# StevenWang30/R-PCC

Hardware: AMD Instinct MI355X
Metric: frames/s (64E, 64x2048 range img), projection->segmentation->model->quantise (higher is better)
Workload: dtype f32

## Files before the change

r-pcc_amd/csrc/rpcc_hip.hip:

```cpp
#include <hip/hip_runtime.h>
#include <limits.h>
#include <math.h>
#include <stdint.h>
#include <stdio.h>
#include <string.h>

#include <algorithm>
#include <mutex>
#include <new>
#include <type_traits>
#include <utility>
#include <vector>
#include "../../include/rpcc_hip.h"
#include "rpcc_device.h"
#include "ref_rules.h"

using namespace rpcc;

static thread_local char g_err[512] = "";
static int set_err(int code, const char *fmt, const char *a = "", const char *b = "") {
    snprintf(g_err, sizeof(g_err), fmt, a, b);
    return code;
}
#define HIP_TRY(expr)                                                                      \
// ... 2281 lines not shown
#pragma unroll
        for (int e = 0; e < ASSIGN_PX; e++) unknown |= live[e] && !(tp[e] >= 0.0f);
        if (__ballot(unknown) == 0ull) {
#pragma unroll
            for (int e = 0; e < ASSIGN_PX; e++) reach = fmaxf(reach, live[e] ? (tp[e] < 1e10f ? tp[e] : inf) : 0.0f);
        } else {
#pragma unroll
            for (int e = 0; e < ASSIGN_PX; e++) reach = fmaxf(reach, live[e] ? assign_reach(r[e], tx[e], ty[e], tz[e], tp[e] < 1e10f ? tp[e] : -1.0f, G) : 0.0f);
        }
        reach = dpp_max_f32_native(reach);
        const bool bounded = reach < inf;
        float my_dmin[NR], upper = inf;
#pragma unroll
        for (int rd = 0; rd < NR; rd++) {
            const int k = rd * 64 + lane;
            my_dmin[rd] = inf;
            if (rd * 64 < M && k < M) {
                const float4 cc = cen4[k];
                const float a0 = lo0 - cc.x, b0 = cc.x - hi0, a1 = lo1 - cc.y, b1 = cc.y - hi1, a2 = lo2 - cc.z, b2 = cc.z - hi2;
                const float g0 = fmaxf(fmaxf(a0, b0), 0.0f), g1 = fmaxf(fmaxf(a1, b1), 0.0f), g2 = fmaxf(fmaxf(a2, b2), 0.0f);
                my_dmin[rd] = (g0 * g0 + g1 * g1) + g2 * g2;
                if (!bounded) {
                    const float f0 = fmaxf(fabsf(a0), fabsf(b0)), f1 = fmaxf(fabsf(a1), fabsf(b1)), f2 = fmaxf(fabsf(a2), fabsf(b2));
                    upper = fminf(upper, (f0 * f0 + f1 * f1) + f2 * f2);
                }
            }
        }
        if (!bounded) upper = dpp_min_f32_native(upper);
        const float cut = (bounded ? reach : upper) * 1.000002f;
        unsigned long long surv_m[NR], surv_any = 0ull;
#pragma unroll
        for (int rd = 0; rd < NR; rd++) { surv_m[rd] = rd * 64 < M ? __ballot(my_dmin[rd] <= cut) : 0ull; surv_any |= surv_m[rd]; }
        if (surv_any == 0ull) {
#pragma unroll
            for (int e = 0; e < ASSIGN_PX; e++)
                if (valid[e]) st_at(seg_b, (uint32_t)p[e] * (uint32_t)sizeof(L), (L)(r[e] == 0.0f ? 1 : 0));
            continue;
        }
        float m1[ASSIGN_PX], m2[ASSIGN_PX];
        int k1[ASSIGN_PX];
        rs_v2f xv[ASSIGN_PX / 2], yv[ASSIGN_PX / 2], zv[ASSIGN_PX / 2];
#pragma unroll
        for (int e = 0; e < ASSIGN_PX; e++) { m1[e] = inf; m2[e] = inf; k1[e] = -1; }
#pragma unroll
        for (int e2 = 0; e2 < ASSIGN_PX / 2; e2++) {
            xv[e2] = rs_v2f{x[2 * e2], x[2 * e2 + 1]}; yv[e2] = rs_v2f{y[2 * e2], y[2 * e2 + 1]}; zv[e2] = rs_v2f{z[2 * e2], z[2 * e2 + 1]};
        }
#pragma unroll
        for (int rd = 0; rd < NR; rd++) {
            if (rd * 64 >= M) break;
            unsigned long long surv = surv_m[rd];
            while (surv) {
                const int k = rd * 64 + (int)__ffsll((long long)surv) - 1;
                surv &= surv - 1ull;
                const float4 cc = cen4[k];
#pragma unroll
                for (int e2 = 0; e2 < ASSIGN_PX / 2; e2++) {
                    const rs_v2f dx = xv[e2] - rs_v2f{cc.x, cc.x}, dy = yv[e2] - rs_v2f{cc.y, cc.y}, dz = zv[e2] - rs_v2f{cc.z, cc.z};
                    const rs_v2f dd = (dx * dx + dy * dy) + dz * dz;
#pragma unroll
                    for (int e1 = 0; e1 < 2; e1++) {
                        const int e = 2 * e2 + e1;
                        const float d2 = e1 ? dd.y : dd.x;
                        const bool lt = d2 < m1[e];
                        m2[e] = __builtin_amdgcn_fmed3f(m1[e], m2[e], d2);
                        k1[e] = lt ? k : k1[e];
                        m1[e] = lt ? d2 : m1[e];
                    }
                }
            }
        }
        int lab[ASSIGN_PX];
#pragma unroll
        for (int e = 0; e < ASSIGN_PX; e++) {
            lab[e] = assign_label(r[e], tx[e], ty[e], tz[e], x[e], y[e], z[e], m1[e], m2[e], k1[e], cen4, G);
            if (r[e] == 0.0f) lab[e] = 1;
            if (valid[e]) st_at(seg_b, (uint32_t)p[e] * (uint32_t)sizeof(L), (L)lab[e]);
        }
        if constexpr (SUMS) {
            int todo[ASSIGN_PX];
#pragma unroll
            for (int e = 0; e < ASSIGN_PX; e++) todo[e] = lab[e] >= 2 ? lab[e] : -1;
            static_assert(ASSIGN_PX == 4, "four pixel slots: round_label");
            uint32_t lo[ASSIGN_PX], hi[ASSIGN_PX];
            bool inexact = false;
            unsigned long long pend[ASSIGN_PX];
#pragma unroll
            for (int e = 0; e < ASSIGN_PX; e++) {
                lo[e] = hi[e] = 0u;
                if (todo[e] >= 2) inexact |= !range_fixed(f2u(r[e]), lo[e], hi[e]);
                pend[e] = __ballot(todo[e] >= 2);
            }
#pragma unroll 1
            while ((pend[0] | pend[1] | pend[2] | pend[3]) != 0ull) {
                const int cur = round_label(todo, pend);
                uint32_t slo = 0u, shi = 0u;
#pragma unroll
                for (int e = 0; e < ASSIGN_PX; e++) {
                    const bool mine = todo[e] == cur;
                    pend[e] &= ~__ballot(mine);
                    slo += mine ? lo[e] : 0u;
                    shi += mine ? hi[e] : 0u;
                }
                slo = dpp_sum_u32(slo); shi = dpp_sum_u32(shi);
                if (lane == 0)
                    atomicAdd(reinterpret_cast<unsigned long long *>(&acc.sums[(int64_t)b * acc.KP + cur]), (unsigned long long)slo + ((unsigned long long)shi << 18));
            }
            if (__any(inexact) && lane == 0) acc.flags[4 * b] = 1;
        }
    }
}

static inline int kpad(int M);
template <class L, class S>
static void launch_assign_form(const float *ri, const float *tm, const double *ground, const float *centers, int B, int H, int W, int M, L *seg,
                               hipStream_t st, const float *temp, const S acc) {
    const int ntile = ((H + ASSIGN_ROWS - 1) / ASSIGN_ROWS) * ((W + 31) / 32);
    const dim3 grid((ntile + ASSIGN_WAVES * ASSIGN_TILES_PER_WAVE - 1) / (ASSIGN_WAVES * ASSIGN_TILES_PER_WAVE), B);
    const size_t sh = (size_t)M * sizeof(float4);
    if constexpr (sizeof(L) == 1) assign_kernel<L, 4><<<grid, 64 * ASSIGN_WAVES, sh, st>>>(ri, tm, ground, centers, H, W, M, seg, temp, acc);
    else if (M <= 510)            assign_kernel<L, 8><<<grid, 64 * ASSIGN_WAVES, sh, st>>>(ri, tm, ground, centers, H, W, M, seg, temp, acc);
    else                          assign_kernel<L, 16><<<grid, 64 * ASSIGN_WAVES, sh, st>>>(ri, tm, ground, centers, H, W, M, seg, temp, acc);
}
template <class L>
static int launch_assign(const float *ri, const float *tm, const double *ground, const float *centers, int B, int H,
                         int W, int M, L *seg, hipStream_t st, const float *temp = nullptr, int64_t *sums = nullptr, int32_t *flags = nullptr) {
    ARG_TRY((sums == nullptr) == (flags == nullptr));
    if (sums != nullptr) launch_assign_form(ri, tm, ground, centers, B, H, W, M, seg, st, temp, LabelSums{sums, flags, kpad(M)});
    else                 launch_assign_form(ri, tm, ground, centers, B, H, W, M, seg, st, temp, NoSums{});
    LAUNCH_CHECK();
    return RPCC_OK;
}

template <class L>
static int assign_entry(const float *ri, const float *tm, const double *ground, const float *centers, int B, int H, int W, int M, L *seg,
                        void *stream) {
    ARG_TRY(B > 0 && B <= RPCC_MAX_BATCH && H > 0 && W > 0 && M > 0 && M <= LabelTraits<L>::max_clusters && ri && tm && ground && centers && seg);
    return launch_assign(ri, tm, ground, centers, B, H, W, M, seg, (hipStream_t)stream);
}
extern "C" int rpcc_assign(const float *ri, const float *tm, const double *ground, const float *centers, int B, int H, int W, int M, uint8_t *seg,
                           void *stream) {
    return assign_entry(ri, tm, ground, centers, B, H, W, M, seg, stream);
}
extern "C" int rpcc_assign_wide(const float *ri, const float *tm, const double *ground, const float *centers, int B, int H, int W, int M, uint16_t *seg,
                                void *stream) {
    return assign_entry(ri, tm, ground, centers, B, H, W, M, seg, stream);
}

#define TILE 1024
#define FX_UNIT_LOG2 28

static inline int kpad(int M) { return ((M + 2) + 63) & ~63; }
static inline int ntiles(int P) { return (P + TILE - 1) / TILE; }
struct WsLayout {
    int64_t *sums;
    int32_t *flags;
    uint32_t *hist;
    size_t bytes;
};
static WsLayout ws_layout(void *ws, int B, int P, int M) {
    const size_t KP = (size_t)kpad(M), T = (size_t)ntiles(P);
    Carve c(ws);
    WsLayout L;
    L.sums = c.take<int64_t>((size_t)B * KP * 8); L.flags = c.take<int32_t>((size_t)B * 4 * 4); L.hist = c.take<uint32_t>((size_t)B * T * KP * 4);
    L.bytes = c.bytes();
    return L;
}
struct PlaneLayout { uint32_t *order; float4 *pts4; size_t bytes; };
static PlaneLayout plane_layout(void *extra, int B, int P) {
    Carve c(extra);
    uint32_t *order = c.take<uint32_t>((size_t)B * P * 4);
    float4 *pts4 = c.take<float4>((size_t)B * P * 16);
    return {order, pts4, c.bytes()};
}
struct BatchLayout {
    WsLayout L;
    int32_t *epoch, *kpn = nullptr; char *proj_scratch, *extra = nullptr; float *temp, *rays_soa, *tiletab, *label_acc = nullptr;
    size_t proj_bytes, bytes;
};
static BatchLayout batch_layout(void *ws, int B, int P, int M, int64_t total_points, bool general) {
    Carve c(ws);
    BatchLayout l;
    l.L = ws_layout(ws, B, P, M); c.take(l.L.bytes); l.epoch = c.take<int32_t>(256);
    l.proj_bytes = round_up(project_layout(nullptr, total_points, B, P).bytes, 256); l.proj_scratch = c.take(l.proj_bytes);
    l.temp = c.take<float>((size_t)B * P * 4);
    l.rays_soa = c.take<float>((size_t)3 * P * 4 + 256, 4);
    l.tiletab = c.take<float>(0, 4);
    const size_t tab_bytes = fps_tab_bound_bytes(B, P), ksz = round_up((size_t)B * (M + 2) * 4, 256);
    Carve t(l.tiletab);
    t.take(tab_bytes + 256);
    if (general) {
        l.extra = t.take(plane_layout(nullptr, B, P).bytes);
        l.kpn = t.take<int32_t>(ksz, 4); l.label_acc = t.take<float>(ksz, 4); t.take(256, 1);
    }
    char *handoff_end = reinterpret_cast<char *>(wc_slot_of(rs_wc_of(reinterpret_cast<int32_t *>(l.tiletab), B, P), B, B).cnt);
    l.bytes = handoff_end <= reinterpret_cast<char *>(l.tiletab) + tab_bytes ? c.bytes() + t.bytes() : 0;
    return l;
}
static size_t batch_ws_bytes(int B, int P, int M, int64_t total_points, bool general) {
    const size_t n = B > 0 && P > 0 && M > 0 ? batch_layout(nullptr, B, P, M, total_points, general).bytes : 0;
    return n ? n + 4096 : 0;
}
extern "C" size_t rpcc_workspace_bytes(int B, int P, int M, int64_t total_points) { return batch_ws_bytes(B, P, M, total_points, false); }
extern "C" size_t rpcc_workspace_bytes_general(int B, int P, int M, int64_t total_points) { return batch_ws_bytes(B, P, M, total_points, true); }

#define SCAN_U 16
#define SCAN_THREADS 256
struct ScanArgs {
    const float *ri;
    const uint8_t *seg;
    const double *ground;
    int P, M, KP, T, KP2;
    const int64_t *sums;
    const int32_t *flags;
    uint32_t *hist;
    float *model;
    int32_t *counts, *nnz;
};
__device__ __forceinline__ void model_scan_body(const ScanArgs &A, const int b) {
    const float *__restrict__ ri = A.ri;
    const uint8_t *__restrict__ seg = A.seg;
    const double *__restrict__ ground = A.ground;
    const int P = A.P, M = A.M, KP = A.KP, T = A.T, KP2 = A.KP2;
    const int64_t *__restrict__ sums = A.sums;
    const int32_t *__restrict__ flags = A.flags;
    uint32_t *__restrict__ hist = A.hist;
    float *__restrict__ model = A.model;
    int32_t *__restrict__ counts = A.counts, *__restrict__ nnz = A.nnz;
    __shared__ uint32_t gtot[SCAN_THREADS];
    __shared__ uint32_t base[256];
    __shared__ uint32_t wsum[4];
    const int K = M + 2;
    const int NG = SCAN_THREADS / KP2, k = threadIdx.x & (KP2 - 1), grp = threadIdx.x / KP2;
    const int TG = (T + NG - 1) / NG, tbeg = grp * TG, tend = min(T, tbeg + TG);
    uint32_t *gh = hist + (int64_t)b * T * KP;
    const uint32_t kp4 = (uint32_t)KP * 4u, k4 = (uint32_t)k * 4u;
    const bool held = TG <= SCAN_U;
    uint32_t c[SCAN_U];
    uint32_t part = 0;
    if (k < K) {
        if (held) {
#pragma unroll
            for (int j = 0; j < SCAN_U; j++) c[j] = ld_at(gh, (uint32_t)min(tbeg + j, T - 1) * kp4 + k4);
#pragma unroll
            for (int j = 0; j < SCAN_U; j++) { if (tbeg + j >= tend) c[j] = 0u; part += c[j]; }
        } else {
            for (int t0 = tbeg; t0 < tend; t0 += SCAN_U) {
                uint32_t d[SCAN_U];
#pragma unroll
                for (int j = 0; j < SCAN_U; j++) d[j] = ld_at(gh, (uint32_t)min(t0 + j, T - 1) * kp4 + k4);
#pragma unroll
                for (int j = 0; j < SCAN_U; j++) part += t0 + j < tend ? d[j] : 0u;
            }
        }
    }
    gtot[grp * KP2 + k] = k < K ? part : 0u;
    __syncthreads();
    uint32_t total = 0;
    for (int g2 = 0; g2 < NG; g2++) total += gtot[g2 * KP2 + k];
    {
        const int kk = threadIdx.x;
        uint32_t v = 0u;
        if (kk < 256 && kk < K && kk != 1) { for (int g2 = 0; g2 < NG; g2++) v += gtot[g2 * KP2 + kk]; }
        const uint32_t incl = dpp_scan_incl_u32(v);
        if (kk < 256 && (kk & 63) == 63) wsum[kk >> 6] = incl;
        __syncthreads();
        if (kk < 256) {
            uint32_t off = 0u;
            for (int w = 0; w < (kk >> 6); w++) off += wsum[w];
            base[kk] = off + incl - v;
            if (kk == 255 && nnz) nnz[b] = (int32_t)(off + incl);
        }
    }
    __syncthreads();
    if (k < K) {
        uint32_t run = base[k];
        for (int g2 = 0; g2 < grp; g2++) run += gtot[g2 * KP2 + k];
        if (held) {
#pragma unroll
            for (int j = 0; j < SCAN_U; j++) {
                if (tbeg + j < tend) { st_at(gh, (uint32_t)(tbeg + j) * kp4 + k4, run); run += c[j]; }
            }
        } else {
            for (int t0 = tbeg; t0 < tend; t0 += SCAN_U) {
                uint32_t d[SCAN_U];
#pragma unroll
                for (int j = 0; j < SCAN_U; j++) d[j] = ld_at(gh, (uint32_t)min(t0 + j, T - 1) * kp4 + k4);
#pragma unroll
                for (int j = 0; j < SCAN_U; j++) {
                    if (t0 + j < tend) { st_at(gh, (uint32_t)(t0 + j) * kp4 + k4, run); run += d[j]; }
                }
            }
        }
        if (counts && grp == 0) counts[(int64_t)b * K + k] = (int32_t)total;
    }
    if (k < K && grp == 0 && model != nullptr)
        point_model_row(model, ground, flags, seg, ri, P, K, b, k, (long long)sums[(int64_t)b * KP + k], total);
}
__global__ __launch_bounds__(SCAN_THREADS) void model_scan_kernel(const ScanArgs A) { model_scan_body(A, blockIdx.x); }
__global__ __launch_bounds__(SCAN_THREADS) void model_scan_multi_kernel(const MultiArgs<ScanArgs> m) {
    int b, t;
    const ScanArgs &A = multi_locate(m, b, t);
    model_scan_body(A, b);
}
#define SCANW_THREADS 1024
template <class L>
__global__ __launch_bounds__(SCANW_THREADS) void model_scan_wide_kernel(const float *__restrict__ ri, const L *__restrict__ seg, const double *__restrict__ ground,
                                                                        int P, int M, int KP, int T, const int64_t *__restrict__ sums,
                                                                        const int32_t *__restrict__ flags, uint32_t *__restrict__ hist,
                                                                        float *__restrict__ model, int32_t *__restrict__ counts, int32_t *__restrict__ nnz) {
    __shared__ uint32_t wsum[SCANW_THREADS / 64];
    const int b = blockIdx.x, k = threadIdx.x, K = M + 2, lane = k & 63, wave = k >> 6;
    uint32_t *gh = hist + (int64_t)b * T * KP;
    const uint32_t kp4 = (uint32_t)KP * 4u, k4 = (uint32_t)min(k, KP - 1) * 4u;
    uint32_t total = 0u;
    for (int t0 = 0; t0 < T; t0 += SCAN_U) {
        uint32_t d[SCAN_U];
#pragma unroll
        for (int j = 0; j < SCAN_U; j++) d[j] = ld_at(gh, (uint32_t)min(t0 + j, T - 1) * kp4 + k4);
#pragma unroll
        for (int j = 0; j < SCAN_U; j++) total += (t0 + j < T && k < K) ? d[j] : 0u;
    }
    const uint32_t v = (k < K && k != 1) ? total : 0u;
    const uint32_t incl = dpp_scan_incl_u32(v);
    if (lane == 63) wsum[wave] = incl;
    __syncthreads();
    uint32_t off = 0u;
    for (int w = 0; w < wave; w++) off += wsum[w];
    if (k == SCANW_THREADS - 1 && nnz) nnz[b] = (int32_t)(off + incl);
    if (k >= K) return;
    uint32_t run = off + incl - v;
    for (int t0 = 0; t0 < T; t0 += SCAN_U) {
        uint32_t d[SCAN_U];
#pragma unroll
        for (int j = 0; j < SCAN_U; j++) d[j] = ld_at(gh, (uint32_t)min(t0 + j, T - 1) * kp4 + k4);
#pragma unroll
        for (int j = 0; j < SCAN_U; j++)
            if (t0 + j < T) { st_at(gh, (uint32_t)(t0 + j) * kp4 + k4, run); run += d[j]; }
    }
    if (counts) counts[(int64_t)b * K + k] = (int32_t)total;
    if (model != nullptr)
        point_model_row(model, ground, flags, seg, ri, P, K, b, k, (long long)sums[(int64_t)b * KP + k], total);
}
template <bool SUMS>
__device__ __forceinline__ void hist_aggregate(const int (&lab)[4], const uint32_t (&rb)[4], const int nval, int KP, int T, int64_t *__restrict__ sums,
                                               int32_t *__restrict__ flags, uint32_t *__restrict__ hist, const int b, const int t);
template <bool VEC, class L = uint8_t, bool SUMS = true>
__device__ __forceinline__ void model_hist_body(const float *__restrict__ ri, const L *__restrict__ seg,
                                                int P, int KP, int T, int64_t *__restrict__ sums,
                                                int32_t *__restrict__ flags, uint32_t *__restrict__ hist, const int b, const int t) {
    const L *seg_b = seg + (int64_t)b * P;
    const float *ri_b = SUMS ? ri + (int64_t)b * P : nullptr;
    const int p0 = t * TILE + 4 * (int)threadIdx.x;
    const int nval = min(max(P - p0, 0), 4);
    int lab[4];
    uint32_t rb[4];
    if (VEC) {
        const uint32_t q = (uint32_t)(nval > 0 ? p0 : 0);
        load_labels4(seg_b, q, lab);
        if constexpr (SUMS) {
            const uint4 r4 = ld_at(reinterpret_cast<const uint4 *>(ri_b), q * 4u);
            rb[0] = r4.x; rb[1] = r4.y; rb[2] = r4.z; rb[3] = r4.w;
        }
    } else {
#pragma unroll
        for (int e = 0; e < 4; e++) {
            const uint32_t gp = (uint32_t)min(p0 + e, P - 1);
            lab[e] = ld_at(seg_b, gp * (uint32_t)sizeof(L));
            if constexpr (SUMS) rb[e] = f2u(ld_at(ri_b, gp * 4u));
        }
    }
    hist_aggregate<SUMS>(lab, rb, nval, KP, T, sums, flags, hist, b, t);
}
template <bool SUMS>
__device__ __forceinline__ void hist_aggregate(const int (&lab)[4], const uint32_t (&rb)[4], const int nval, int KP, int T, int64_t *__restrict__ sums,
                                               int32_t *__restrict__ flags, uint32_t *__restrict__ hist, const int b, const int t) {
    extern __shared__ __attribute__((aligned(16))) unsigned char smem_raw[];
    unsigned long long *ssum = reinterpret_cast<unsigned long long *>(smem_raw);
    uint32_t *scnt = reinterpret_cast<uint32_t *>(SUMS ? smem_raw + (size_t)KP * 8 : smem_raw);
    const int lane = threadIdx.x & 63;
    for (int k = threadIdx.x; k < KP; k += blockDim.x) {
        if constexpr (SUMS) ssum[k] = 0ull;
        scnt[k] = 0u;
    }
    __syncthreads();
    bool inexact = false;
    int todo[4];
    uint32_t lo[4], hi[4];
#pragma unroll
    for (int e = 0; e < 4; e++) {
        todo[e] = e < nval ? lab[e] : -1;
        lo[e] = hi[e] = 0u;
        if constexpr (SUMS) {
            if (todo[e] >= 2) inexact |= !range_fixed(rb[e], lo[e], hi[e]);
        }
    }
#define HIST_ROUNDS 3
    unsigned long long pend[4];
#pragma unroll
    for (int e = 0; e < 4; e++) pend[e] = __ballot(todo[e] >= 0);
#pragma unroll 1
    for (int round = 0; round < HIST_ROUNDS && (pend[0] | pend[1] | pend[2] | pend[3]) != 0ull; round++) {
        const int cur = round_label(todo, pend);
        int ctot = 0;
        uint32_t slo = 0u, shi = 0u;
#pragma unroll
        for (int e = 0; e < 4; e++) {
            const bool mine = todo[e] == cur;
            const unsigned long long m = __ballot(mine);
            ctot += (int)__popcll(m);
            pend[e] &= ~m;
            if constexpr (SUMS) { slo += mine ? lo[e] : 0u; shi += mine ? hi[e] : 0u; }
        }
        const bool sum = SUMS && cur >= 2;
        if (sum) { slo = dpp_sum_u32(slo); shi = dpp_sum_u32(shi); }
        if (lane == 0) {
            atomicAdd(&scnt[cur], (uint32_t)ctot);
            if (sum) atomicAdd(&ssum[cur], (unsigned long long)slo + ((unsigned long long)shi << 18));
        }
    }
#pragma unroll
    for (int e = 0; e < 4; e++) {
        if (pend[e] != 0ull && ((pend[e] >> lane) & 1ull)) {
            atomicAdd(&scnt[todo[e]], 1u);
            if constexpr (SUMS) {
                if (todo[e] >= 2) atomicAdd(&ssum[todo[e]], (unsigned long long)lo[e] + ((unsigned long long)hi[e] << 18));
            }
        }
    }
    if constexpr (SUMS) {
        if (__any(inexact) && lane == 0) flags[4 * b] = 1;
    }
    __syncthreads();
    for (int k = threadIdx.x; k < KP; k += blockDim.x) {
        hist[((int64_t)b * T + t) * KP + k] = scnt[k];
        if constexpr (SUMS) {
            if (ssum[k]) atomicAdd(reinterpret_cast<unsigned long long *>(&sums[(int64_t)b * KP + k]), ssum[k]);
        }
    }
}
template <bool VEC, class L = uint8_t, bool SUMS = true>
__global__ __launch_bounds__(256) void model_hist_kernel(const float *__restrict__ ri, const L *__restrict__ seg,
                                                         int P, int KP, int T, int64_t *__restrict__ sums,
                                                         int32_t *__restrict__ flags, uint32_t *__restrict__ hist) {
    model_hist_body<VEC, L, SUMS>(ri, seg, P, KP, T, sums, flags, hist, blockIdx.y, blockIdx.x);
}
struct HistGroup {
    const uint8_t *seg;
    int P, T, vec;
    uint32_t *hist;
};
__global__ __launch_bounds__(256) void model_hist_multi_kernel(const MultiArgs<HistGroup> m, int KP) {
    int b, t;
    const HistGroup &a = multi_locate(m, b, t);
    if (a.vec) model_hist_body<true, uint8_t, false>(nullptr, a.seg, a.P, KP, a.T, nullptr, nullptr, a.hist, b, t);
    else       model_hist_body<false, uint8_t, false>(nullptr, a.seg, a.P, KP, a.T, nullptr, nullptr, a.hist, b, t);
}
static inline size_t hist_lds_bytes(int KP, bool sums) { return (sums ? (size_t)KP * 8 : 0) + (size_t)KP * 4; }
template <class L>
static inline bool hist_vec(int P, const L *seg, const float *ri) { return (P & 3) == 0 && seg4_aligned(seg) && (ri == nullptr || aligned16(ri)); }
static inline int scan_kp2(int M) { int v = 1; while (v < M + 2) v <<= 1; return v; }
template <class L>
static int launch_hist_scan(const float *ri, const L *seg, const double *ground, int B, int P, int M, const WsLayout &lay, float *model,
                            int32_t *counts, int32_t *nnz, hipStream_t st, bool summed = false, bool counted = false) {
    const int KP = kpad(M), T = ntiles(P);
    const bool hist_sums = ri != nullptr && !summed;
    const size_t sh = hist_lds_bytes(KP, hist_sums);
    const bool vec = hist_vec(P, seg, hist_sums ? ri : nullptr);
    if (counted) {
    } else if (hist_sums) {
        if (vec) model_hist_kernel<true, L, true><<<dim3(T, B), 256, sh, st>>>(ri, seg, P, KP, T, lay.sums, lay.flags, lay.hist);
        else     model_hist_kernel<false, L, true><<<dim3(T, B), 256, sh, st>>>(ri, seg, P, KP, T, lay.sums, lay.flags, lay.hist);
    } else {
        if (vec) model_hist_kernel<true, L, false><<<dim3(T, B), 256, sh, st>>>(nullptr, seg, P, KP, T, nullptr, nullptr, lay.hist);
        else     model_hist_kernel<false, L, false><<<dim3(T, B), 256, sh, st>>>(nullptr, seg, P, KP, T, nullptr, nullptr, lay.hist);
    }
    LAUNCH_CHECK();
    if constexpr (sizeof(L) == 1) {
        const ScanArgs sa = {ri, seg, ground, P, M, KP, T, scan_kp2(M), lay.sums, lay.flags, lay.hist, model, counts, nnz};
        model_scan_kernel<<<B, SCAN_THREADS, 0, st>>>(sa);
    } else {
        model_scan_wide_kernel<L><<<B, SCANW_THREADS, 0, st>>>(ri, seg, ground, P, M, KP, T, lay.sums, lay.flags, lay.hist, model, counts, nnz);
    }
    LAUNCH_CHECK();
    return RPCC_OK;
}

template <class L>
static int launch_point_model(const float *ri, const L *seg, const double *ground, int B, int P, int M,
                              float *model, int32_t *counts, int32_t *nnz, void *ws, hipStream_t st, bool cleared = false, bool summed = false,
                              bool counted = false) {
    const WsLayout lay = ws_layout(ws, B, P, M);
    if (!cleared) HIP_TRY(hipMemsetAsync(lay.sums, 0, (size_t)((char *)lay.hist - (char *)lay.sums), st));
    return launch_hist_scan(ri, seg, ground, B, P, M, lay, model, counts, nnz, st, summed, counted);
}

template <class L>
static int point_model_entry(const float *ri, const L *seg, const double *ground, int B, int P, int M, float *model, int32_t *counts,
                             void *ws, void *stream) {
    ARG_TRY(B > 0 && B <= RPCC_MAX_BATCH && P > 0 && M > 0 && M <= LabelTraits<L>::max_clusters && ri && seg && ground && model && ws);
    return launch_point_model(ri, seg, ground, B, P, M, model, counts, nullptr, ws, (hipStream_t)stream);
}
extern "C" int rpcc_point_model(const float *ri, const uint8_t *seg, const double *ground, int B, int P, int M, float *model, int32_t *counts, void *ws,
                                void *stream) {
    return point_model_entry(ri, seg, ground, B, P, M, model, counts, ws, stream);
}
extern "C" int rpcc_point_model_wide(const float *ri, const uint16_t *seg, const double *ground, int B, int P, int M, float *model, int32_t *counts, void *ws,
                                     void *stream) {
    return point_model_entry(ri, seg, ground, B, P, M, model, counts, ws, stream);
}

__device__ __forceinline__ void segment_prefix(uint32_t *segcnt, int SEGP, const uint32_t *tile_off, int K) {
    const int row = threadIdx.x >> 4, sgi = threadIdx.x & 15;
    for (int k0 = 0; k0 < K; k0 += 16) {
        const int k = k0 + row;
        const bool ok = k < K;
        const uint32_t c = ok ? segcnt[sgi * SEGP + k] : 0u;
        uint32_t v = c;
        v += (uint32_t)__builtin_amdgcn_update_dpp(0, (int)v, 0x111, 0xf, 0xf, false);
        v += (uint32_t)__builtin_amdgcn_update_dpp(0, (int)v, 0x112, 0xf, 0xf, false);
        v += (uint32_t)__builtin_amdgcn_update_dpp(0, (int)v, 0x114, 0xf, 0xf, false);
        v += (uint32_t)__builtin_amdgcn_update_dpp(0, (int)v, 0x118, 0xf, 0xf, false);
        if (ok) segcnt[sgi * SEGP + k] = tile_off[k] + v - c;
    }
}
__device__ __forceinline__ int segment_rank(int j, int lab, uint32_t *segcnt, int SEGP) {
    const int lane = threadIdx.x & 63, wave = threadIdx.x >> 6;
    int rank = 0, todo = lab;
    while (true) {
        const unsigned long long pending = __ballot(todo >= 0);
        if (!pending) break;
        const int leader = (int)__ffsll((long long)pending) - 1;
        const int cur = __builtin_amdgcn_readlane(todo, leader);
        const unsigned long long same = __ballot(todo == cur);
        if (todo == cur) {
            rank = __popcll(same & ((1ull << lane) - 1ull));
            if (lane == leader) segcnt[(j * 4 + wave) * SEGP + cur] = (uint32_t)__popcll(same);
            todo = -1;
        }
    }
    return rank;
}
__device__ __forceinline__ void segment_offsets(uint32_t *segcnt, int SEGP, const uint32_t *tile_off, int K) {
    __syncthreads();
    segment_prefix(segcnt, SEGP, tile_off, K);
    __syncthreads();
}
__device__ __forceinline__ uint32_t segment_slot(int j, int lab, int rank, const uint32_t *segcnt, int SEGP) {
    return segcnt[(j * 4 + (int)(threadIdx.x >> 6)) * SEGP + lab] + (uint32_t)rank;
}
static inline size_t segment_lds_bytes(int KP) { return (size_t)16 * (KP + 1) * 4 + (size_t)KP * 4; }

template <bool RESIDUAL_ONLY, bool VEC, class L = uint8_t>
__device__ __forceinline__ void predict_quantize_body(const float *__restrict__ ri, const float *__restrict__ tm,
                                                      const L *__restrict__ seg,
                                                      const float *__restrict__ model,
                                                      const uint32_t *__restrict__ hist, float acc,
                                                      const float *__restrict__ label_acc,
                                                      const float *__restrict__ residual_in, int P, int M,
                                                      int KP, int T, int16_t *__restrict__ q16,
                                                      int32_t *__restrict__ q32, float *__restrict__ pred_out,
                                                      int32_t *__restrict__ epoch_inc, const int b, const int t) {
    extern __shared__ __attribute__((aligned(16))) unsigned char smem_raw[];
    if (epoch_inc && b == 0 && t == 0 && threadIdx.x == 0) *epoch_inc += 1;
    float4 *smodel = reinterpret_cast<float4 *>(smem_raw);
    uint32_t *wcnt = reinterpret_cast<uint32_t *>(smodel + KP);
    uint32_t *soff = wcnt + 4 * KP;
    float *sacc = reinterpret_cast<float *>(soff + KP);
    const int K = M + 2;
    const int lane = threadIdx.x & 63, wave = threadIdx.x >> 6;
    seg += (int64_t)b * P;
    if (!RESIDUAL_ONLY) ri += (int64_t)b * P;
    if (residual_in) residual_in += (int64_t)b * P;
    if (pred_out) pred_out += (int64_t)b * P;
    if (q16) q16 += (int64_t)b * P;
    if (q32) q32 += (int64_t)b * P;
    if (label_acc) label_acc += (int64_t)b * K;
    if (!RESIDUAL_ONLY) model += (int64_t)b * K * 4;
    hist += ((int64_t)b * T + t) * KP;
    const int p0 = t * TILE + 4 * (int)threadIdx.x;
    const int nval = min(max(P - p0, 0), 4);
    int lab[4];
    float rv[4], ray[12], rin[4];
    if (VEC) {
        const uint32_t q = (uint32_t)(nval > 0 ? p0 : 0);
        load_labels4(seg, q, lab);
        if (RESIDUAL_ONLY) {
#pragma unroll
            for (int e = 0; e < 4; e++) rv[e] = 0.0f;
#pragma unroll
            for (int i = 0; i < 12; i++) ray[i] = 0.0f;
        } else {
            const float4 r4 = ld_at(reinterpret_cast<const float4 *>(ri), q * 4u);
            rv[0] = r4.x; rv[1] = r4.y; rv[2] = r4.z; rv[3] = r4.w;
            const float4 a = ld_at(reinterpret_cast<const float4 *>(tm), q * 12u), bq = ld_at(reinterpret_cast<const float4 *>(tm), q * 12u + 16u),
                         c = ld_at(reinterpret_cast<const float4 *>(tm), q * 12u + 32u);
            ray[0] = a.x; ray[1] = a.y; ray[2] = a.z; ray[3] = a.w; ray[4] = bq.x; ray[5] = bq.y; ray[6] = bq.z; ray[7] = bq.w;
            ray[8] = c.x; ray[9] = c.y; ray[10] = c.z; ray[11] = c.w;
        }
        if (residual_in) {
            const float4 x4 = ld_at(reinterpret_cast<const float4 *>(residual_in), q * 4u);
            rin[0] = x4.x; rin[1] = x4.y; rin[2] = x4.z; rin[3] = x4.w;
        } else {
            rin[0] = rin[1] = rin[2] = rin[3] = 0.0f;
        }
    } else {
#pragma unroll
        for (int e = 0; e < 4; e++) {
            const uint32_t up = (uint32_t)min(p0 + e, P - 1);
            lab[e] = ld_at(seg, up * (uint32_t)sizeof(L));
            rv[e] = RESIDUAL_ONLY ? 0.0f : ld_at(ri, up * 4u);
            if (RESIDUAL_ONLY) { ray[3 * e] = ray[3 * e + 1] = ray[3 * e + 2] = 0.0f; }
            else { ray[3 * e] = ld_f32(tm, up * 12u); ray[3 * e + 1] = ld_f32(tm, up * 12u + 4u); ray[3 * e + 2] = ld_f32(tm, up * 12u + 8u); }
            rin[e] = residual_in ? ld_at(residual_in, up * 4u) : 0.0f;
        }
    }
    for (uint32_t i = threadIdx.x; i < (uint32_t)K; i += 256u) {
        smodel[i] = RESIDUAL_ONLY ? make_float4(0.f, 0.f, 0.f, 0.f) : make_float4(model[4 * i], model[4 * i + 1], model[4 * i + 2], model[4 * i + 3]);
        soff[i] = hist[i];
        if (label_acc) sacc[i] = label_acc[i];
        wcnt[i] = 0u; wcnt[KP + i] = 0u; wcnt[2 * KP + i] = 0u; wcnt[3 * KP + i] = 0u;
// ... 426 lines not shown
                                 io->counts, p.ws, p.extra, st);
    case ST_QUANTISE:
        if (io->nonuniform) {
            const rpcc_nonuniform_cfg *nu = io->nonuniform;
            if ((rc = launch_features(io->ri, seg, Bs, p.g.H, p.g.W, nu->feature_region, nu->segments, nu->sharp_num, nu->less_sharp_num,
                                      nu->flat_num, nullptr, io->key_point_map, st, p.kpn, M + 2)))
                return rc;
            if ((rc = launch_salience_levels<L>(io->counts, p.kpn, Bs, M, salience_params(nu->levels, nu->level_kp_num, nu->level_acc, nu->ground_level),
                                                io->salience, p.label_acc, st)))
                return rc;
        }
        return launch_predict_quantize(io->ri, io->tm, seg, io->model, p.acc, p.label_acc, nullptr, Bs, P, M, io->q16,
                                       nullptr, nullptr, p.ws, st, p.epoch);
    }
    return RPCC_ERR_ARG;
}

static int check_batch_io(const rpcc_batch_io *io, int B, rpcc_geom g, int M, const void *ws, bool wide = false) {
    ARG_TRY(io != nullptr && ws != nullptr && B > 0 && B <= RPCC_MAX_BATCH && M > 0 && M <= (wide ? RPCC_MAX_CLUSTERS_WIDE : RPCC_MAX_CLUSTERS) &&
            g.H > 1 && g.W > 0);
    ARG_TRY(io->offsets && io->tm && io->ground && io->ri && io->seg && io->cen_pix && io->centers && io->model &&
            io->counts && io->q16 && io->nnz && io->info);
    ARG_TRY((io->flags & ~(RPCC_FPS_BRUTEFORCE | RPCC_FPS_MODE_BITS)) == 0);
    const int P = g.H * g.W;
    if (wide)
        ARG_TRY(!(io->flags & RPCC_FPS_MODE_BITS));
    else
        ARG_TRY(P % 4 == 0 || fps_pick_range(g.H, g.W, B, io->flags, true, true).family != FPS_ONE_PASS);
    ARG_TRY(io->model_method == 0 || io->model_method == 1);
    ARG_TRY(point_floats(io->point_stride_bytes) > 0 && (io->point_stride_bytes != 16 || (reinterpret_cast<uintptr_t>(io->xyz) & 15u) == 0));
    if (io->nonuniform) {
        const rpcc_nonuniform_cfg *nu = io->nonuniform;
        ARG_TRY(io->salience && io->key_point_map && nu->levels >= 1 && nu->levels <= 8 && nu->ground_level >= 0 && nu->ground_level < nu->levels);
    }
    return RPCC_OK;
}

template <class L>
static int run_batch(const rpcc_batch_io *io, int B, rpcc_geom g, int M, double ground_threshold, float acc, void *ws, int stage_mask, hipStream_t st,
                     const void *beams = nullptr) {
    BatchPlan p;
    int rc;
    if ((rc = plan_batch(p, io, B, io->total, g, M, ground_threshold, acc, reinterpret_cast<char *>(ws)))) return rc;
    p.beams = beams;
    for (int stage = 0; stage < ST_COUNT; stage++)
        if (((stage_mask >> stage) & 1) && (rc = run_stage<L>(p, stage, st))) return rc;
    return RPCC_OK;
}

extern "C" int rpcc_compress_batch(const rpcc_batch_io *io, int B, rpcc_geom g, int M, double ground_threshold,
                                   float acc, void *ws, void *stream) {
    int rc;
    if ((rc = check_batch_io(io, B, g, M, ws))) return rc;
    return run_batch<uint8_t>(io, B, g, M, ground_threshold, acc, ws, (1 << ST_COUNT) - 1, (hipStream_t)stream);
}

extern "C" int rpcc_compress_batch_stages(const rpcc_batch_io *io, int B, rpcc_geom g, int M, double ground_threshold, float acc, void *ws,
                                          int stage_mask, void *stream) {
    int rc;
    if ((rc = check_batch_io(io, B, g, M, ws))) return rc;
    return run_batch<uint8_t>(io, B, g, M, ground_threshold, acc, ws, stage_mask, (hipStream_t)stream);
}

static int mixed_ground(const BatchPlan *pl, int G, hipStream_t st) {
    RansacMulti m;
    m.n = 0; m.first[0] = 0;
    for (int i = 0; i < G; i++) {
        if (!pl[i].fit_ground) continue;
        const rpcc_batch_io *io = pl[i].io;
        m.a[m.n] = {io->ri, io->tm, pl[i].P, (uint32_t)io->ground_seed, io->ground, pl[i].zcnt, io->frame_ids,
                    pl[i].zcnt ? rs_wc_of(pl[i].zcnt, pl[i].Bs, pl[i].P) : nullptr, 100};
        m.first[m.n + 1] = m.first[m.n] + pl[i].Bs;
        m.n++;
    }
    if (m.n == 0) return RPCC_OK;
    return launch_ground_ransac_multi(m, st);
}
static int mixed_fps(const BatchPlan *pl, int G, hipStream_t st) {
    int rc, total = 0, tt = FPS_TT_SMALL;
    for (int i = 0; i < G; i++)
        if (pl[i].tiled && pl[i].io->timer == nullptr) total += pl[i].Bs;
    bool common[RPCC_MAX_GROUPS];
    FpsMulti m;
    m.n = 0; m.first[0] = 0;
    for (int i = 0; i < G; i++) {
        const BatchPlan &p = pl[i];
        const FpsPick k = fps_pick_range(p.g.H, p.g.W, total, p.io->flags, range_quads16(p.g.W, p.io->ri, p.temp, p.io->tm), true);
        common[i] = k.family == FPS_PLANAR && p.io->timer == nullptr;
        if (!common[i]) continue;
        tt = k.threads;
        m.a[m.n] = {p.io->ri, p.io->tm, p.temp, p.io->info, fps_tiling_range(p.g.H, p.g.W), p.io->cen_pix, p.io->centers, p.tiletab, p.rays_soa};
        m.edge[m.n] = k.unaligned ? 1 : 0;
        m.first[m.n + 1] = m.first[m.n] + p.Bs;
        m.n++;
    }
    if (m.n > 0) {
        if (tt == FPS_TT_SMALL) fps_regtab_planar_multi_kernel<FPS_TT_SMALL><<<m.first[m.n], FPS_TT_SMALL, 0, st>>>(m, pl[0].M, 0);
        else                    fps_regtab_planar_multi_kernel<FPS_TT_BATCH><<<m.first[m.n], FPS_TT_BATCH, 0, st>>>(m, pl[0].M, 0);
        LAUNCH_CHECK();
    }
    for (int i = 0; i < G; i++)
        if (!common[i] && (rc = run_stage<uint8_t>(pl[i], ST_FPS, st))) return rc;
    return RPCC_OK;
}
static int mixed_planes(const BatchPlan *pl, int G, hipStream_t st) {
    PlaneMulti m;
    m.n = 0; m.first[0] = 0;
    const int M = pl[0].M, K = M + 2, wpg = PL_THREADS / 64, groups = (K + wpg - 1) / wpg;
    for (int i = 0; i < G; i++) {
        const BatchPlan &p = pl[i];
        if (p.io->model_method == 0) continue;
        m.a[m.n] = plane_group_args(p.io->tm, p.io->ground, p.Bs, p.P, M, p.io->plane_cos_cut, (uint32_t)p.io->plane_seed, p.io->frame_ids,
                                    p.io->model, p.io->counts, p.ws, p.extra, nullptr);
        m.first[m.n + 1] = m.first[m.n] + p.Bs * (K - 2) + p.Bs * groups;
        m.n++;
    }
    if (m.n == 0) return RPCC_OK;
    plane_model_multi_kernel<10><<<m.first[m.n], PL_THREADS, 0, st>>>(m, M, kpad(M), PL_BIG);
    LAUNCH_CHECK();
    return RPCC_OK;
}

template <class A>
static void multi_add(MultiArgs<A> &m, const A &a, int frames, int per_frame) {
    m.a[m.n] = a; m.per[m.n] = per_frame; m.first[m.n + 1] = m.first[m.n] + frames * per_frame; m.n++;
}
static int mixed_assign(const BatchPlan *pl, int G, hipStream_t st) {
    int rc;
    for (int i = 0; i < G; i++) {
        const rpcc_batch_io *io = pl[i].io;
        const bool point = io->model_method == 0;
        if ((rc = launch_assign(io->ri, io->tm, io->ground, io->centers, pl[i].Bs, pl[i].g.H, pl[i].g.W, pl[i].M, io->seg, st,
                                (io->flags & RPCC_FPS_MODE_BITS) ? nullptr : pl[i].temp, point ? pl[i].L.sums : nullptr,
                                point ? pl[i].L.flags : nullptr))) return rc;
    }
    return RPCC_OK;
}
static int mixed_labels(const BatchPlan *pl, int G, hipStream_t st) {
    const int M = pl[0].M, KP = kpad(M);
    MultiArgs<HistGroup> mh; MultiArgs<ScanArgs> ms; MultiArgs<OrderGroup> mo;
    mh.n = ms.n = mo.n = 0; mh.first[0] = ms.first[0] = mo.first[0] = 0;
    for (int i = 0; i < G; i++) {
        const BatchPlan &p = pl[i];
        const rpcc_batch_io *io = p.io;
        const int T = ntiles(p.P);
        const bool point = io->model_method == 0;
        const float *ri = point ? io->ri : nullptr;
        multi_add(mh, HistGroup{io->seg, p.P, T, hist_vec(p.P, io->seg, (const float *)nullptr) ? 1 : 0, p.L.hist}, p.Bs, T);
        multi_add(ms, ScanArgs{ri, io->seg, point ? io->ground : nullptr, p.P, M, KP, T, scan_kp2(M), p.L.sums, p.L.flags, p.L.hist,
                               point ? io->model : nullptr, io->counts, io->nnz}, p.Bs, 1);
        const PlaneLayout pa = plane_layout(p.extra, p.Bs, p.P);
        if (!point) multi_add(mo, OrderGroup{io->seg, p.L.hist, p.P, T, pa.order, io->ri, io->tm, pa.pts4}, p.Bs, T);
    }
    model_hist_multi_kernel<<<mh.first[mh.n], 256, hist_lds_bytes(KP, false), st>>>(mh, KP);
    LAUNCH_CHECK();
    model_scan_multi_kernel<<<ms.first[ms.n], SCAN_THREADS, 0, st>>>(ms);
    LAUNCH_CHECK();
    if (mo.n > 0) {
        label_order_multi_kernel<<<mo.first[mo.n], 256, label_order_lds_bytes(KP), st>>>(mo, M, KP);
        LAUNCH_CHECK();
    }
    return RPCC_OK;
}
static int mixed_quantise(const BatchPlan *pl, int G, hipStream_t st) {
    int rc;
    const int M = pl[0].M, KP = kpad(M);
    MultiArgs<SalienceGroup> msal; MultiArgs<QuantGroup> mq;
    msal.n = mq.n = 0; msal.first[0] = mq.first[0] = 0;
    for (int i = 0; i < G; i++) {
        const BatchPlan &p = pl[i];
        const rpcc_batch_io *io = p.io;
        if (io->nonuniform) {
            const rpcc_nonuniform_cfg *nu = io->nonuniform;
            if ((rc = launch_features(io->ri, io->seg, p.Bs, p.g.H, p.g.W, nu->feature_region, nu->segments, nu->sharp_num, nu->less_sharp_num,
                                      nu->flat_num, nullptr, io->key_point_map, st, p.kpn, M + 2)))
                return rc;
            multi_add(msal, SalienceGroup{io->counts, p.kpn, salience_params(nu->levels, nu->level_kp_num, nu->level_acc, nu->ground_level), io->salience,
                                          p.label_acc}, p.Bs, 1);
        }
        const int T = ntiles(p.P);
        const bool vec = quantise_vec(p.P, io->seg, io->ri, io->tm, nullptr, false);
        multi_add(mq, QuantGroup{io->ri, io->tm, io->model, p.label_acc, io->seg, p.L.hist, p.P, T, vec ? 1 : 0, io->q16, p.epoch}, p.Bs, T);
    }
    if (msal.n > 0) {
        salience_levels_multi_kernel<<<msal.first[msal.n], 256, 0, st>>>(msal, M);
        LAUNCH_CHECK();
    }
    predict_quantize_multi_kernel<<<mq.first[mq.n], 256, quantise_lds_bytes(KP), st>>>(mq, pl[0].acc, M, KP);
    LAUNCH_CHECK();
    return RPCC_OK;
}

extern "C" int rpcc_compress_batch_mixed(const rpcc_batch_io *ios, const int *Bs, const rpcc_geom *geoms, int G, int M,
                                         double ground_threshold, float acc, void *const *wss, void *stream) {
    ARG_TRY(ios != nullptr && Bs != nullptr && geoms != nullptr && wss != nullptr && G >= 1 && G <= RPCC_MAX_GROUPS);
    int rc;
    BatchPlan pl[RPCC_MAX_GROUPS];
    for (int i = 0; i < G; i++) {
        if ((rc = check_batch_io(&ios[i], Bs[i], geoms[i], M, wss[i]))) return rc;
        if ((rc = plan_batch(pl[i], &ios[i], Bs[i], ios[i].total, geoms[i], M, ground_threshold, acc, reinterpret_cast<char *>(wss[i])))) return rc;
    }
    hipStream_t st = (hipStream_t)stream;
    for (int stage = 0; stage < ST_COUNT; stage++) {
        if (stage == ST_GROUND) rc = mixed_ground(pl, G, st);
        else if (stage == ST_FPS) rc = mixed_fps(pl, G, st);
        else if (stage == ST_PLANES) rc = mixed_planes(pl, G, st);
        else if (stage == ST_ASSIGN_LABELS) { if (!(rc = mixed_assign(pl, G, st))) rc = mixed_labels(pl, G, st); }
        else if (stage == ST_QUANTISE) rc = mixed_quantise(pl, G, st);
        else
            for (int i = 0; i < G && !(rc = run_stage<uint8_t>(pl[i], stage, st)); i++) {}
        if (rc) return rc;
    }
    return RPCC_OK;
}

#include "wide_kernels.h"

static bool mid_clusters_ok(const rpcc_batch_io *io, rpcc_geom g, int M) {
    (void)io;
    return M <= RPCC_MAX_CLUSTERS_MID && fps_prunable(fps_tiling_range(g.H, g.W));
}

struct WideWs {
    uint32_t *keys_in, *vals_in, *keys_out, *vals_out, *order, *base; int32_t *pos, *kpn, *flags; float4 *pts4, *cen4; unsigned long long *sums;
    float *label_acc, *temp, *tiletab; char *proj; void *sort_tmp; size_t proj_bytes, sort_bytes, bytes;
};
static size_t wide_sort_bytes(int64_t n, int end_bit) {
    size_t b = 0;
    uint32_t *z = nullptr;
    (void)rocprim::radix_sort_pairs(nullptr, b, z, z, z, z, (size_t)n, 0u, (unsigned)end_bit, (hipStream_t)0);
    return b;
}
static inline int wide_key_bits(int B) { int v = 16; while ((1 << (v - 16)) < B) v++; return v; }
static WideWs wide_layout(void *ws, int B, int P, int M, int64_t total_points) {
    WideWs w;
    const size_t BP = (size_t)B * P, K = (size_t)M + 2;
    Carve c(ws);
    w.keys_in = c.take<uint32_t>(BP * 4); w.vals_in = c.take<uint32_t>(BP * 4); w.keys_out = c.take<uint32_t>(BP * 4); w.vals_out = c.take<uint32_t>(BP * 4);
    w.pos = c.take<int32_t>(BP * 4); w.order = c.take<uint32_t>(BP * 4); w.pts4 = c.take<float4>(BP * 16);
    w.sums = c.take<unsigned long long>((size_t)B * K * 8); w.base = c.take<uint32_t>((size_t)B * K * 4); w.kpn = c.take<int32_t>((size_t)B * K * 4);
    w.label_acc = c.take<float>((size_t)B * K * 4); w.flags = c.take<int32_t>((size_t)B * 16); w.cen4 = c.take<float4>((size_t)B * M * 16);
    w.temp = c.take<float>(BP * 4); w.tiletab = c.take<float>(fps_tab_bound_bytes(B, P));
    w.proj_bytes = round_up(project_layout(nullptr, total_points, B, P).bytes, 256); w.proj = c.take(w.proj_bytes);
    w.sort_bytes = wide_sort_bytes((int64_t)BP, wide_key_bits(B)); w.sort_tmp = c.take(w.sort_bytes + 256);
    w.bytes = round_up(c.bytes(), 256);
    return w;
}
extern "C" size_t rpcc_wide_workspace_bytes(int B, int P, int M, int64_t total_points) {
    if (B <= 0 || P <= 0 || M <= 0) return 0;
    const size_t sorted = wide_layout(nullptr, B, P, M, total_points).bytes + 4096;
    return M <= RPCC_MAX_CLUSTERS_MID ? std::max(sorted, rpcc_workspace_bytes_general(B, P, M, total_points)) : sorted;
}
template <class L>
static int wide_order(const L *seg, const float *ri_for_sums, const float *ri, const float *tm, int B, int P, int M, const WideWs &w, int32_t *counts,
                      int32_t *nnz, bool want_pts, hipStream_t st) {
    const int K = M + 2;
    const int64_t n = (int64_t)B * P;
    HIP_TRY(hipMemsetAsync(counts, 0, (size_t)B * K * 4, st));
    HIP_TRY(hipMemsetAsync(w.sums, 0, (size_t)B * K * 8, st));
    HIP_TRY(hipMemsetAsync(w.flags, 0, (size_t)B * 16, st));
    wide_keys_kernel<L><<<dim3((P + 255) / 256, B), 256, 0, st>>>(seg, ri_for_sums, P, K, w.keys_in, w.vals_in, counts, w.sums, w.flags);
    LAUNCH_CHECK();
    size_t sb = w.sort_bytes;
    HIP_TRY(rocprim::radix_sort_pairs(w.sort_tmp, sb, w.keys_in, w.keys_out, w.vals_in, w.vals_out, (size_t)n, 0u, (unsigned)wide_key_bits(B), st));
    wide_bases_kernel<<<B, 256, 0, st>>>(counts, K, w.base, nnz);
    wide_positions_kernel<<<(unsigned)((n + 255) / 256), 256, 0, st>>>(w.keys_out, w.vals_out, counts, P, K, n, w.pos, w.order, ri, tm, want_pts ? w.pts4 : nullptr);
    LAUNCH_CHECK();
    return RPCC_OK;
}

extern "C" int rpcc_compress_batch_wide(const rpcc_batch_io *io, int B, rpcc_geom g, int M, double ground_threshold, float acc, void *ws, void *stream) {
    int rc;
    if ((rc = check_batch_io(io, B, g, M, ws, true))) return rc;
    hipStream_t st = (hipStream_t)stream;
    const int P = g.H * g.W, K = M + 2;
    ARG_TRY(fps_prunable(fps_tiling_range(g.H, g.W)));
    if (mid_clusters_ok(io, g, M)) return run_batch<uint16_t>(io, B, g, M, ground_threshold, acc, ws, (1 << ST_COUNT) - 1, st);
    const WideWs w = wide_layout(ws, B, P, M, io->total);
    uint16_t *seg = reinterpret_cast<uint16_t *>(io->seg);
    if ((rc = launch_project(io->xyz, io->offsets, io->total, 0, B, g, io->ri, w.proj, w.proj_bytes, st, nullptr, nullptr, nullptr, nullptr,
                             point_floats(io->point_stride_bytes)))) return rc;
    if (io->ground_seed >= 0 && (rc = launch_ground_ransac(io->ri, io->tm, B, P, (uint32_t)io->ground_seed, false, io->ground, nullptr, st, nullptr, io->frame_ids))) return rc;
    const bool brute = (io->flags & RPCC_FPS_BRUTEFORCE) != 0;
    if ((rc = launch_ground_mask(io->ri, io->tm, io->ground, ground_threshold, B, g.H, g.W, w.temp, io->info, brute ? nullptr : w.tiletab, st, false))) return rc;
    if ((rc = launch_fps_range(io->ri, io->tm, w.temp, io->info, B, g.H, g.W, M, io->cen_pix, io->centers, io->flags, false, brute ? nullptr : w.tiletab, nullptr, st))) return rc;
    const bool point = io->model_method == 0;
    wide_cen4_kernel<<<(B * M + 255) / 256, 256, 0, st>>>(io->centers, B * M, w.cen4);
    wide_assign_kernel<<<dim3((P + 255) / 256, B), 256, 0, st>>>(io->ri, io->tm, io->ground, w.cen4, P, M, seg);
    LAUNCH_CHECK();
    if ((rc = wide_order<uint16_t>(seg, point ? io->ri : nullptr, io->ri, io->tm, B, P, M, w, io->counts, io->nnz, !point, st))) return rc;
    if (point) {
        wide_point_model_kernel<uint16_t><<<dim3((K + 255) / 256, B), 256, 0, st>>>(io->ri, seg, io->ground, io->counts, w.sums, w.flags, P, K, io->model);
        LAUNCH_CHECK();
    } else {
        PlaneParams pp;
        pp.cos_cut = io->plane_cos_cut; pp.thr = 0.1f; pp.min_points = 30; pp.iters = 10; pp.seed = (uint32_t)io->plane_seed; pp.frame_ids = io->frame_ids; pp.inject = nullptr;
        const int wpg = PL_THREADS / 64, groups = (K + wpg - 1) / wpg;
        plane_model_kernel<10><<<B * (K - 2) + B * groups, PL_THREADS, 0, st>>>(io->tm, w.order, w.pts4, w.base, io->counts, io->ground, B, P, M, K, 1, pp, PL_BIG, io->model);
        LAUNCH_CHECK();
    }
    const float *label_acc = nullptr;
    if (io->nonuniform) {
        const rpcc_nonuniform_cfg *nu = io->nonuniform;
        HIP_TRY(hipMemsetAsync(w.kpn, 0, (size_t)B * K * 4, st));
        if ((rc = launch_features<uint16_t>(io->ri, seg, B, g.H, g.W, nu->feature_region, nu->segments, nu->sharp_num, nu->less_sharp_num, nu->flat_num,
                                            nullptr, io->key_point_map, st, w.kpn, K))) return rc;
        if ((rc = launch_salience_levels<uint16_t>(io->counts, w.kpn, B, M, salience_params(nu->levels, nu->level_kp_num, nu->level_acc, nu->ground_level),
                                                   io->salience, w.label_acc, st)))
            return rc;
        label_acc = w.label_acc;
// ... 199 lines not shown
```

Before: 372,800.

## Fuse per-tile label counting into scan kernel using LDS packed 16-bit counts

Adds a fused count+scan kernel that computes per-tile label histograms directly into LDS, using packed 16-bit counters and SWAR byte-matching. The per-tile counts are then scanned from LDS, so the separate histogram kernel launch and its global histogram round trip go away. It is used when the model sums are not needed and the table fits in 96KB of LDS. In exchange, one block per frame does all the counting, which reduces parallelism compared with the T×B grid, and the scan is forced onto its non-held path.

```diff
diff --git a/r-pcc_amd/csrc/label_bytes.h b/r-pcc_amd/csrc/label_bytes.h
--- /dev/null
+++ b/r-pcc_amd/csrc/label_bytes.h
@@ -0,0 +1,25 @@
+#ifndef RPCC_LABEL_BYTES_H
+#define RPCC_LABEL_BYTES_H
+
+#include <stdint.h>
+
+#if defined(__HIPCC__) || defined(__CUDACC__)
+#define RPCC_LB_FN __host__ __device__ static inline __attribute__((always_inline))
+#else
+#define RPCC_LB_FN static inline
+#endif
+
+RPCC_LB_FN uint32_t rpcc_label_eq_bytes(uint32_t w, uint32_t label) {
+    const uint32_t y = w ^ (label * 0x01010101u);
+    return ~(((y & 0x7F7F7F7Fu) + 0x7F7F7F7Fu) | y) & 0x80808080u;
+}
+
+RPCC_LB_FN uint32_t rpcc_label_count_word(uint32_t w, uint32_t label, uint32_t *pending) {
+    const uint32_t eq = rpcc_label_eq_bytes(w, label) & *pending;
+    *pending ^= eq;
+    return (uint32_t)__builtin_popcount(eq);
+}
+
+RPCC_LB_FN uint32_t rpcc_label_marks(int n) { return n >= 4 ? 0x80808080u : n <= 0 ? 0u : (0x80808080u & ((1u << (8 * n)) - 1u)); }
+
+#endif
diff --git a/r-pcc_amd/csrc/rpcc_hip.hip b/r-pcc_amd/csrc/rpcc_hip.hip
--- a/r-pcc_amd/csrc/rpcc_hip.hip
+++ b/r-pcc_amd/csrc/rpcc_hip.hip
@@ -2457,6 +2457,7 @@
 
 static inline int kpad(int M) { return ((M + 2) + 63) & ~63; }
 static inline int ntiles(int P) { return (P + TILE - 1) / TILE; }
+__host__ __device__ static inline int count_row_words(int K) { return (K + 1) >> 1; }
 struct WsLayout {
     int64_t *sums;
     int32_t *flags;
@@ -2522,6 +2523,7 @@
     float *model;
     int32_t *counts, *nnz;
 };
+template <bool LDS_COUNTS = false, int NT = SCAN_THREADS>
 __device__ __forceinline__ void model_scan_body(const ScanArgs &A, const int b) {
     const float *__restrict__ ri = A.ri;
     const uint8_t *__restrict__ seg = A.seg;
@@ -2532,28 +2534,34 @@
     uint32_t *__restrict__ hist = A.hist;
     float *__restrict__ model = A.model;
     int32_t *__restrict__ counts = A.counts, *__restrict__ nnz = A.nnz;
-    __shared__ uint32_t gtot[SCAN_THREADS];
+    __shared__ uint32_t gtot[NT];
     __shared__ uint32_t base[256];
     __shared__ uint32_t wsum[4];
     const int K = M + 2;
-    const int NG = SCAN_THREADS / KP2, k = threadIdx.x & (KP2 - 1), grp = threadIdx.x / KP2;
+    const int NG = NT / KP2, k = threadIdx.x & (KP2 - 1), grp = threadIdx.x / KP2;
     const int TG = (T + NG - 1) / NG, tbeg = grp * TG, tend = min(T, tbeg + TG);
     uint32_t *gh = hist + (int64_t)b * T * KP;
     const uint32_t kp4 = (uint32_t)KP * 4u, k4 = (uint32_t)k * 4u;
-    const bool held = TG <= SCAN_U;
+    const bool held = !LDS_COUNTS && TG <= SCAN_U;
+    extern __shared__ __attribute__((aligned(16))) unsigned char smem_raw[];
+    const uint32_t row2 = (uint32_t)count_row_words(K) * 4u, k2 = (uint32_t)k * 2u;
+    auto count_at = [&](int t) -> uint32_t {
+        if constexpr (LDS_COUNTS) return (uint32_t)ld_at(reinterpret_cast<const uint16_t *>(smem_raw), (uint32_t)t * row2 + k2);
+        else return ld_at(gh, (uint32_t)t * kp4 + k4);
+    };
     uint32_t c[SCAN_U];
     uint32_t part = 0;
     if (k < K) {
         if (held) {
 #pragma unroll
-            for (int j = 0; j < SCAN_U; j++) c[j] = ld_at(gh, (uint32_t)min(tbeg + j, T - 1) * kp4 + k4);
+            for (int j = 0; j < SCAN_U; j++) c[j] = count_at(min(tbeg + j, T - 1));
 #pragma unroll
             for (int j = 0; j < SCAN_U; j++) { if (tbeg + j >= tend) c[j] = 0u; part += c[j]; }
         } else {
             for (int t0 = tbeg; t0 < tend; t0 += SCAN_U) {
                 uint32_t d[SCAN_U];
 #pragma unroll
-                for (int j = 0; j < SCAN_U; j++) d[j] = ld_at(gh, (uint32_t)min(t0 + j, T - 1) * kp4 + k4);
+                for (int j = 0; j < SCAN_U; j++) d[j] = count_at(min(t0 + j, T - 1));
 #pragma unroll
                 for (int j = 0; j < SCAN_U; j++) part += t0 + j < tend ? d[j] : 0u;
             }
@@ -2590,7 +2598,7 @@
             for (int t0 = tbeg; t0 < tend; t0 += SCAN_U) {
                 uint32_t d[SCAN_U];
 #pragma unroll
-                for (int j = 0; j < SCAN_U; j++) d[j] = ld_at(gh, (uint32_t)min(t0 + j, T - 1) * kp4 + k4);
+                for (int j = 0; j < SCAN_U; j++) d[j] = count_at(min(t0 + j, T - 1));
 #pragma unroll
                 for (int j = 0; j < SCAN_U; j++) {
                     if (t0 + j < tend) { st_at(gh, (uint32_t)(t0 + j) * kp4 + k4, run); run += d[j]; }
@@ -2608,6 +2616,63 @@
     const ScanArgs &A = multi_locate(m, b, t);
     model_scan_body(A, b);
 }
+#include "label_bytes.h"
+#define COUNT_U 8
+#define COUNT_SCAN_THREADS 512
+template <bool WHOLE>
+__device__ __forceinline__ void count_tile_row(const uint32_t w0, const uint32_t w1, const uint32_t w2, const uint32_t w3, const int nval, const int K,
+                                               uint32_t *row) {
+    uint32_t p0 = rpcc_label_marks(WHOLE ? 4 : nval), p1 = rpcc_label_marks(WHOLE ? 4 : nval - 4), p2 = rpcc_label_marks(WHOLE ? 4 : nval - 8),
+             p3 = rpcc_label_marks(WHOLE ? 4 : nval - 12);
+    while ((p0 | p1 | p2 | p3) != 0u) {
+        const uint32_t px = p0 ? p0 : p1 ? p1 : p2 ? p2 : p3, wx = p0 ? w0 : p1 ? w1 : p2 ? w2 : w3;
+        const uint32_t cur = (wx >> (__ffs((int)px) - 8)) & 255u;
+        const uint32_t n = rpcc_label_count_word(w0, cur, &p0) + rpcc_label_count_word(w1, cur, &p1) + rpcc_label_count_word(w2, cur, &p2) +
+                           rpcc_label_count_word(w3, cur, &p3);
+        if ((int)cur < K) atomicAdd(&row[cur >> 1], n << (16u * (cur & 1u)));
+    }
+}
+template <int NT>
+__device__ __forceinline__ void count_tiles_lds(const uint8_t *__restrict__ seg_b, const int P, const int T, const int K) {
+    extern __shared__ __attribute__((aligned(16))) unsigned char smem_raw[];
+    uint32_t *tab = reinterpret_cast<uint32_t *>(smem_raw);
+    const int RW = count_row_words(K), lane = threadIdx.x & 63, wave = threadIdx.x >> 6, NW = NT / 64;
+    for (int i = threadIdx.x; i < (T * RW + 3) >> 2; i += NT) reinterpret_cast<uint4 *>(tab)[i] = make_uint4(0u, 0u, 0u, 0u);
+    __syncthreads();
+    const int Tw = ((uintptr_t)seg_b & 15u) == 0 ? P / TILE : 0;
+    for (int t0 = wave; t0 < Tw; t0 += NW * COUNT_U) {
+        uint4 x[COUNT_U];
+#pragma unroll
+        for (int j = 0; j < COUNT_U; j++)
+            x[j] = ld_at(reinterpret_cast<const uint4 *>(seg_b), (uint32_t)min(t0 + NW * j, Tw - 1) * (uint32_t)TILE + 16u * (uint32_t)lane);
+#pragma unroll
+        for (int j = 0; j < COUNT_U; j++) {
+            const int t = t0 + NW * j;
+            if (t < Tw) count_tile_row<true>(x[j].x, x[j].y, x[j].z, x[j].w, 16, K, tab + t * RW);
+        }
+    }
+    for (int t = Tw + wave; t < T; t += NW) {
+        const int p0 = t * TILE + 16 * lane, nval = min(max(P - p0, 0), 16);
+        uint32_t w[4] = {0u, 0u, 0u, 0u};
+#pragma unroll
+        for (int e = 0; e < 16; e++) w[e >> 2] |= (uint32_t)ld_at(seg_b, (uint32_t)min(p0 + e, P - 1)) << (8 * (e & 3));
+        count_tile_row<false>(w[0], w[1], w[2], w[3], nval, K, tab + t * RW);
+    }
+    __syncthreads();
+}
+__global__ __launch_bounds__(COUNT_SCAN_THREADS) void count_scan_kernel(const ScanArgs A) {
+    count_tiles_lds<COUNT_SCAN_THREADS>(A.seg + (int64_t)blockIdx.x * A.P, A.P, A.T, A.M + 2);
+    model_scan_body<true, COUNT_SCAN_THREADS>(A, blockIdx.x);
+}
+__global__ __launch_bounds__(COUNT_SCAN_THREADS) void count_scan_multi_kernel(const MultiArgs<ScanArgs> m) {
+    int b, t;
+    const ScanArgs &A = multi_locate(m, b, t);
+    count_tiles_lds<COUNT_SCAN_THREADS>(A.seg + (int64_t)b * A.P, A.P, A.T, A.M + 2);
+    model_scan_body<true, COUNT_SCAN_THREADS>(A, b);
+}
+static inline size_t count_scan_lds_budget() { return (size_t)96 * 1024; }
+static inline size_t count_scan_lds_bytes(int P, int M) { return round_up((size_t)ntiles(P) * count_row_words(M + 2) * 4, 16); }
+static inline bool count_scan_fits(int P, int M) { return count_scan_lds_bytes(P, M) <= count_scan_lds_budget(); }
 #define SCANW_THREADS 1024
 template <class L>
 __global__ __launch_bounds__(SCANW_THREADS) void model_scan_wide_kernel(const float *__restrict__ ri, const L *__restrict__ seg, const double *__restrict__ ground,
@@ -2769,9 +2834,19 @@
 static int launch_hist_scan(const float *ri, const L *seg, const double *ground, int B, int P, int M, const WsLayout &lay, float *model,
                             int32_t *counts, int32_t *nnz, hipStream_t st, bool summed = false, bool counted = false) {
     const int KP = kpad(M), T = ntiles(P);
-    const bool hist_sums = ri != nullptr && !summed;
+    const bool hist_sums = ri != nullptr && model != nullptr && !summed;
     const size_t sh = hist_lds_bytes(KP, hist_sums);
     const bool vec = hist_vec(P, seg, hist_sums ? ri : nullptr);
+    if constexpr (sizeof(L) == 1) {
+        if (!counted && !hist_sums && count_scan_fits(P, M)) {
+            const size_t ch = count_scan_lds_bytes(P, M);
+            const ScanArgs sa = {ri, seg, ground, P, M, KP, T, scan_kp2(M), lay.sums, lay.flags, lay.hist, model, counts, nnz};
+            HIP_TRY(ensure_dyn_lds(reinterpret_cast<const void *>(&count_scan_kernel), (int)ch));
+            count_scan_kernel<<<B, COUNT_SCAN_THREADS, ch, st>>>(sa);
+            LAUNCH_CHECK();
+            return RPCC_OK;
+        }
+    }
     if (counted) {
     } else if (hist_sums) {
         if (vec) model_hist_kernel<true, L, true><<<dim3(T, B), 256, sh, st>>>(ri, seg, P, KP, T, lay.sums, lay.flags, lay.hist);
@@ -3504,10 +3579,19 @@
         const PlaneLayout pa = plane_layout(p.extra, p.Bs, p.P);
         if (!point) multi_add(mo, OrderGroup{io->seg, p.L.hist, p.P, T, pa.order, io->ri, io->tm, pa.pts4}, p.Bs, T);
     }
-    model_hist_multi_kernel<<<mh.first[mh.n], 256, hist_lds_bytes(KP, false), st>>>(mh, KP);
-    LAUNCH_CHECK();
-    model_scan_multi_kernel<<<ms.first[ms.n], SCAN_THREADS, 0, st>>>(ms);
-    LAUNCH_CHECK();
+    size_t ch = 0;
+    bool fits = true;
+    for (int i = 0; i < G; i++) { fits = fits && count_scan_fits(pl[i].P, M); ch = std::max(ch, count_scan_lds_bytes(pl[i].P, M)); }
+    if (fits) {
+        HIP_TRY(ensure_dyn_lds(reinterpret_cast<const void *>(&count_scan_multi_kernel), (int)ch));
+        count_scan_multi_kernel<<<ms.first[ms.n], COUNT_SCAN_THREADS, ch, st>>>(ms);
+        LAUNCH_CHECK();
+    } else {
+        model_hist_multi_kernel<<<mh.first[mh.n], 256, hist_lds_bytes(KP, false), st>>>(mh, KP);
+        LAUNCH_CHECK();
+        model_scan_multi_kernel<<<ms.first[ms.n], SCAN_THREADS, 0, st>>>(ms);
+        LAUNCH_CHECK();
+    }
     if (mo.n > 0) {
         label_order_multi_kernel<<<mo.first[mo.n], 256, label_order_lds_bytes(KP), st>>>(mo, M, KP);
         LAUNCH_CHECK();
```

Result: faster. 382,200, median of 6 (+2.5%).
